# martinjrobins/diffsol

Measured on AMD Instinct MI355X. Metric: ODE steps/sec (and Newton solves/sec) per ensemble, higher is better.
Workload: dtype f64

## Files before the change

diffsol_amd/csrc/dsh_adaptive.hip:

```cpp
#include <cmath>
#include <cstdio>
#include <vector>

#include <cstring>
#include <map>
#include <mutex>
#include <vector>

#include "dsh_internal.hpp"
#include "dsh_resident.hpp"

#ifdef DSH_EXPERIMENTS
#include <hipcub/hipcub.hpp>
#endif
#include "dsh_adaptive_kernel.hpp"
#ifdef DSH_EXPERIMENTS
#include "dsh_member_sched_kernel.hpp"
#endif
#include "dsh_jit.hpp"

using namespace dsh;


extern "C" {

int dsh_experiments_enabled(void) {
#ifdef DSH_EXPERIMENTS
  return 1;
#else
  return 0;
#endif
}

void dsh_adaptive_default_options(dsh_adaptive_options* o) {
  if (!o) return;
#define DSH_X(T, name, value) o->name = value;
  DSH_ADAPTIVE_BODY_OPTIONS(DSH_X)
#undef DSH_X
  o->ic_use_linesearch = 1;
  o->ic_max_linesearch_iterations = 10;
  o->ic_max_linear_solver_setups = 4;
  o->ic_max_newton_iterations = 10;
  o->ic_step_reduction_factor = 0.5;
  o->ic_armijo_constant = 1e-4;
  o->deterministic_pow = 1;
  o->group = 1;
}

int dsh_model_has_adaptive(int model, int64_t size) {
  if (is_jit_model(model)) {
    const JitInfo* ji = jit_info(model);
    if (!ji) return 0;
    return (ji->form == DSH_JIT_FORM_STATIC && ji->n <= 4) || (ji->form == DSH_JIT_FORM_STATIC_BANDED && ji->n <= 512) ? 1 : 0;
  }
  bool ok = false;
  dispatch_static_model(model, size, [&](auto mdl) {
    using Mdl = decltype(mdl);
    ok = Mdl::N <= 4;
  });
  return ok ? 1 : 0;
}

}
namespace dsh {
bool adaptive_fast_launch(int model, int64_t size, bool ba, bool wave, const dsh_adaptive_options& opts, dim3 grid, hipStream_t stream, int64_t nb, const double* p,
                          const double* atol, const AdaptiveConsts* consts, const double* t_eval, double* y_out, int32_t* stats, int32_t* status, double* t_root,
                          int32_t* root_idx, int32_t* ncols, unsigned long long* totals);
}
namespace {
struct SensSpec { double* out; double rtol; const double* atol_host; int64_t natol; };
template <class Mdl> constexpr bool adaptive_sens_ok() {
  if constexpr (model_has_sens<Mdl>::value) return Mdl::N <= 4 && !Mdl::HAS_MASS && Mdl::NROOTS == 0 && model_band_k<Mdl>::value == 0;
  else return false;
}
struct StepsSpec { double* t_out; int64_t cap; };
int bdf_solve_adaptive_impl(dsh_ctx* ctx, int model, int64_t size, int64_t nb, const double* p, const double* atol, int64_t atol_nb, double rtol, double t0,
                            double h0, const dsh_adaptive_options* opts, const double* t_eval_host, int64_t n_eval, double* y_out, int32_t* stats, int32_t* status,
                            double* t_root, int32_t* root_idx, int32_t* ncols, int64_t* totals_host, const SensSpec* sens, const StepsSpec* steps = nullptr);
}
extern "C" {
int dsh_model_has_adaptive_reset(int model, int64_t size) {
  if (is_jit_model(model)) {
    const JitInfo* ji = jit_info(model);
    if (!(ji && ji->has_reset && ji->nroots > 0)) return 0;
    return (ji->form == DSH_JIT_FORM_STATIC && ji->n <= 4) || (ji->form == DSH_JIT_FORM_STATIC_BANDED && !ji->has_mass) ? 1 : 0;
  }
  bool ok = false;
  dispatch_static_model(model, size, [&](auto mdl) {
    using Mdl = decltype(mdl);
    ok = model_has_reset<Mdl>::value && Mdl::N <= 4 && Mdl::NROOTS > 0 && model_band_k<Mdl>::value == 0;
  });
  return ok ? 1 : 0;
}
int dsh_model_has_adaptive_sens(int model, int64_t size) {
  if (is_jit_model(model)) {
    const JitInfo* ji = jit_info(model);
    if (!(ji && ji->has_sens && !ji->has_mass && ji->nroots == 0)) return 0;
    return (ji->form == DSH_JIT_FORM_STATIC && ji->n <= 4) || ji->form == DSH_JIT_FORM_STATIC_BANDED ? 1 : 0;
  }
  bool ok = false;
  dispatch_static_model(model, size, [&](auto mdl) { ok = adaptive_sens_ok<decltype(mdl)>(); });
  return ok ? 1 : 0;
}
int dsh_bdf_solve_adaptive(dsh_ctx* ctx, int model, int64_t size, int64_t nb, const double* p, const double* atol, int64_t atol_nb, double rtol, double t0,
                           double h0, const dsh_adaptive_options* opts, const double* t_eval_host, int64_t n_eval, double* y_out, int32_t* stats, int32_t* status,
                           double* t_root, int32_t* root_idx, int32_t* ncols, int64_t* totals_host) {
  DSH_ENTER(ctx);
  return bdf_solve_adaptive_impl(ctx, model, size, nb, p, atol, atol_nb, rtol, t0, h0, opts, t_eval_host, n_eval, y_out, stats, status, t_root, root_idx, ncols, totals_host, nullptr);
}
int dsh_bdf_solve_adaptive_sens(dsh_ctx* ctx, int model, int64_t size, int64_t nb, const double* p, const double* atol, int64_t atol_nb, double rtol, double t0,
                                double h0, const dsh_adaptive_options* opts, const double* t_eval_host, int64_t n_eval, double sens_rtol, const double* sens_atol_host,
                                int64_t nsens_atol, double* y_out, double* sens_out, int32_t* stats, int32_t* status, int64_t* totals_host) {
  DSH_ENTER(ctx);
  DSH_REQUIRE(sens_out != nullptr, "sens_out is null");
  DSH_REQUIRE(nsens_atol == 0 || sens_atol_host != nullptr, "sens_atol is null");
  if (!dsh_model_has_adaptive_sens(model, size)) {
    set_error("dsh_bdf_solve_adaptive_sens: the model has no device-resident BDF with forward sensitivities (identity-mass ODE model with parameter derivatives and no root functions: register-resident n <= 4, or the banded lane-per-member form)");
    return DSH_E_UNSUPPORTED;
  }
  const SensSpec sp{sens_out, sens_rtol, sens_atol_host, nsens_atol};
  return bdf_solve_adaptive_impl(ctx, model, size, nb, p, atol, atol_nb, rtol, t0, h0, opts, t_eval_host, n_eval, y_out, stats, status, nullptr, nullptr, nullptr, totals_host, &sp);
}
int dsh_model_has_adaptive_steps(int model, int64_t size) {
  if (!dsh_model_has_adaptive(model, size)) return 0;
  if (is_jit_model(model)) { const JitInfo* ji = jit_info(model); return ji && (ji->form == DSH_JIT_FORM_STATIC || ji->form == DSH_JIT_FORM_STATIC_BANDED) ? 1 : 0; }
  return 1;
}
int dsh_bdf_solve_adaptive_steps(dsh_ctx* ctx, int model, int64_t size, int64_t nb, const double* p, const double* atol, int64_t atol_nb, double rtol, double t0,
                                 double h0, const dsh_adaptive_options* opts, double t_final, int64_t max_cols, double* y_out, double* t_out, int32_t* stats,
                                 int32_t* status, double* t_root, int32_t* root_idx, int32_t* ncols, int64_t* totals_host) {
  DSH_ENTER(ctx);
  DSH_REQUIRE(max_cols >= 2 && max_cols <= 0x7fffffff && y_out != nullptr && t_out != nullptr && ncols != nullptr, "dsh_bdf_solve_adaptive_steps: max_cols >= 2, y_out, t_out and ncols are needed");
  if (!dsh_model_has_adaptive_steps(model, size)) {
    set_error("dsh_bdf_solve_adaptive_steps: the model has neither a register-resident BDF (static model, n <= 4) nor a banded lane-per-member form (the wavefront / workgroup forms have dsh_bdf_solve_wave_member_steps)");
    return DSH_E_UNSUPPORTED;
  }
  const StepsSpec st{t_out, max_cols};
  return bdf_solve_adaptive_impl(ctx, model, size, nb, p, atol, atol_nb, rtol, t0, h0, opts, &t_final, 1, y_out, stats, status, t_root, root_idx, ncols, totals_host, nullptr, &st);
}
}
namespace {
int bdf_solve_adaptive_impl(dsh_ctx* ctx, int model, int64_t size, int64_t nb, const double* p, const double* atol, int64_t atol_nb, double rtol, double t0,
                            double h0, const dsh_adaptive_options* opts, const double* t_eval_host, int64_t n_eval, double* y_out, int32_t* stats, int32_t* status,
                            double* t_root, int32_t* root_idx, int32_t* ncols, int64_t* totals_host, const SensSpec* sens, const StepsSpec* steps) {
  DSH_REQUIRE(ctx != nullptr, "ctx is null");
  DSH_REQUIRE(n_eval >= 1 && t_eval_host != nullptr, "t_eval must hold at least one time");
  DSH_REQUIRE(atol_nb == 1 || atol_nb == nb, "atol must be broadcast (nbatch 1) or per member");
  for (int64_t k = 0; k + 1 < n_eval; ++k) DSH_REQUIRE(t_eval_host[k] <= t_eval_host[k + 1], "t_eval must be increasing (InvalidTEval)");
  DSH_REQUIRE(t_eval_host[0] >= t0, "t_eval[0] before t0 (InvalidTEval)");
  if (!dsh_model_has_adaptive(model, size)) { set_error("dsh_bdf_solve_adaptive: model has no device-resident kernel (needs a static model, n <= 4)"); return DSH_E_UNSUPPORTED; }
  if (nb == 0) return DSH_OK;
  AdaptiveConsts C;
  std::memset((void*)&C, 0, sizeof C);
  C.r.rtol = rtol; C.r.t0 = t0; C.r.h0 = h0; C.r.n_eval = (int)n_eval; C.r.member_lanes = 0;
  C.r.ls_steptol = std::pow(2.220446049250313e-16, 2.0 / 3.0);
  if (opts) C.r.o = *opts; else dsh_adaptive_default_options(&C.r.o);
  if (C.r.o.max_steps <= 0) C.r.o.max_steps = 10000000;
  DSH_REQUIRE(C.r.o.group == 1 || C.r.o.group == 64, "adaptive group must be 1 (per member) or 64 (wavefront lock-step)");
  {
    static const int member_lanes_env = [] { const char* e = std::getenv("DSH_MEMBER_LANES"); const int v = e && *e ? std::atoi(e) : 0; return (v == 8 || v == 16 || v == 32) ? v : 0; }();
    C.r.member_lanes = (C.r.o.group == 1 && !is_jit_model(model) && !sens && !steps) ? member_lanes_env : 0;
  }
  if (steps) { C.steps_t_out = steps->t_out; C.steps_cap = (int)steps->cap; }
  if (sens) {
    C.sens_out = sens->out; C.sens_rtol = sens->rtol; C.sens_error_control = sens->natol > 0 ? 1 : 0;
    int64_t ns = 0, npar_ = 0, nroots_ = 0; int hm_ = 0;
    if (dsh_model_info(model, size, &ns, &npar_, &hm_, &nroots_) != DSH_OK) return DSH_E_INVALID;
    DSH_REQUIRE(sens->natol == 0 || sens->natol == 1 || sens->natol == ns, "sens_atol must have length 1 or nstates");
    bool uniform = true;
    for (int64_t i = 1; i < sens->natol; ++i) uniform = uniform && sens->atol_host[i] == sens->atol_host[0];
    DSH_REQUIRE(ns <= 4 || uniform, "device-resident sensitivities of models with more than 4 states take one sens_atol for every state");
    C.sens_pad = (ns > 4 || sens->natol <= 1) ? 1 : 0;
    for (int64_t i = 0; i < 4 && i < ns; ++i) C.sens_atol[i] = sens->natol == 0 ? 0.0 : (sens->natol == 1 ? sens->atol_host[0] : sens->atol_host[i]);
  }
  {
    const BdfTables T = bdf_new_tables();
    for (int i = 0; i <= kMaxOrder; ++i) { C.alpha[i] = T.alpha[i]; C.gamma[i] = T.gamma[i]; C.ec2[i] = T.ec2[i]; }
    C.r.eta_reset = std::pow(20.0, 1.25);
    C.r.eta_reset_ts = std::pow(100.0, 1.25);
    C.eta_reset_p08 = dsh_det_pow(C.r.eta_reset, 0.8);
    C.eta_reset_ts_p08 = dsh_det_pow(C.r.eta_reset_ts, 0.8);
    for (int ord = 1; ord <= kMaxOrder; ++ord) {
      double* U = C.u[ord - 1];
      for (int k = 0; k < 36; ++k) U[k] = 0.0;
      for (int j = 0; j <= ord; ++j) U[j * 6 + 0] = 1.0;
      for (int j = 1; j <= ord; ++j)
        for (int i = 1; i <= ord; ++i) U[j * 6 + i] = U[j * 6 + i - 1] * ((double)i - 1.0 - 1.0 * (double)j) / (double)i;
    }
  }
  double* t_eval_dev = nullptr;
  unsigned long long* totals_dev = nullptr;
  AdaptiveConsts* consts_dev = nullptr;
  int rc = DSH_OK;
  const size_t cbytes = sizeof(AdaptiveConsts), tbytes = sizeof(double) * (size_t)n_eval, need = cbytes + tbytes;
  bool cached = false;
  if (tbytes <= 4096) {
    if (!ctx->const_cache_dev && hipMalloc((void**)&ctx->const_cache_dev, cbytes + 4096) != hipSuccess) { (void)hipGetLastError(); ctx->const_cache_dev = nullptr; }
    if (ctx->const_cache_dev) {
      if (!ctx->const_cache_host) ctx->const_cache_host = new std::vector<unsigned char>();
      std::vector<unsigned char>& held = *ctx->const_cache_host;
      std::vector<unsigned char> now(need);
      std::memcpy(now.data(), &C, cbytes);
      std::memcpy(now.data() + cbytes, t_eval_host, tbytes);
      if (now != held) {
        held.swap(now);
        DSH_HIP_CHECK(hipMemcpyAsync(ctx->const_cache_dev, held.data(), need, hipMemcpyHostToDevice, ctx->stream));
        DSH_HIP_CHECK(hipStreamSynchronize(ctx->stream));
      }
      consts_dev = (AdaptiveConsts*)ctx->const_cache_dev;
      t_eval_dev = (double*)(ctx->const_cache_dev + cbytes);
      cached = true;
    }
  }
  if (!cached) {
    rc = dsh_malloc(ctx, (int64_t)sizeof(AdaptiveConsts), 0, (void**)&consts_dev);
    if (rc != DSH_OK) return rc;
    DSH_HIP_CHECK(hipMemcpyAsync(consts_dev, &C, sizeof(AdaptiveConsts), hipMemcpyHostToDevice, ctx->stream));
    rc = dsh_malloc(ctx, (int64_t)(sizeof(double) * n_eval), 0, (void**)&t_eval_dev);
    if (rc != DSH_OK) return rc;
    DSH_HIP_CHECK(hipMemcpyAsync(t_eval_dev, t_eval_host, sizeof(double) * n_eval, hipMemcpyHostToDevice, ctx->stream));
  }
  rc = dsh_malloc(ctx, (int64_t)(sizeof(unsigned long long) * 8), 1, (void**)&totals_dev);
  if (rc != DSH_OK) { if (!cached) { dsh_free(ctx, t_eval_dev); dsh_free(ctx, consts_dev); } return rc; }
  const bool ba = atol_nb == 1 && nb != 1;
  const int per_wave = C.r.member_lanes > 0 ? C.r.member_lanes : 64;
  const dim3 grid((unsigned)((nb + per_wave - 1) / per_wave)), blk(64);
  bool launched = false;
  DSH_HIP_CHECK(timing_begin(ctx));
#ifdef DSH_EXPERIMENTS
  const int rebin = [] { const char* e = std::getenv("DSH_REBIN"); return e && *e ? std::atoi(e) : 0; }();
  const int rebin_steps = [] { const char* e = std::getenv("DSH_REBIN_STEPS"); return e && *e ? std::atoi(e) : 0; }();
  if (!sens && !steps && (rebin_steps > 0 || (rebin > 0 && n_eval > rebin)) && !is_jit_model(model) && C.r.o.group == 1 && nb >= 128) {
    double* seg_dbl = nullptr; int* seg_int = nullptr; unsigned long long *keys = nullptr, *keys_out = nullptr; int *idx_iota = nullptr, *lane_member = nullptr; void* cub_tmp = nullptr;
    AdaptiveConsts* seg_consts = nullptr; unsigned int* remaining = nullptr;
    size_t cub_bytes = 0;
    auto release = [&]() { (void)hipFree(seg_dbl); (void)hipFree(seg_int); (void)hipFree(keys); (void)hipFree(keys_out); (void)hipFree(idx_iota); (void)hipFree(lane_member); (void)hipFree(cub_tmp); (void)hipFree(seg_consts); (void)hipFree(remaining); };
    (void)hipcub::DeviceRadixSort::SortPairs(nullptr, cub_bytes, keys, keys_out, idx_iota, lane_member, (int)nb, 0, 64, ctx->stream);
    const bool by_steps = rebin_steps > 0;
    const int nseg = by_steps ? 3 : (int)((n_eval + rebin - 1) / rebin);
    bool okm = hipMalloc((void**)&seg_dbl, sizeof(double) * (size_t)kSegDbl * nb) == hipSuccess && hipMalloc((void**)&seg_int, sizeof(int) * (size_t)kSegInt * nb) == hipSuccess &&
               hipMalloc((void**)&keys, 8 * (size_t)nb) == hipSuccess && hipMalloc((void**)&keys_out, 8 * (size_t)nb) == hipSuccess && hipMalloc((void**)&idx_iota, 4 * (size_t)nb) == hipSuccess &&
               hipMalloc((void**)&lane_member, 4 * (size_t)nb) == hipSuccess && hipMalloc(&cub_tmp, cub_bytes ? cub_bytes : 8) == hipSuccess &&
               hipMalloc((void**)&seg_consts, sizeof(AdaptiveConsts) * (size_t)nseg) == hipSuccess && hipMalloc((void**)&remaining, 4) == hipSuccess;
    if (!okm) { (void)hipGetLastError(); release(); set_error("dsh_bdf_solve_adaptive (DSH_REBIN): out of device memory for the segment state"); dsh_free(ctx, totals_dev); if (!cached) { dsh_free(ctx, t_eval_dev); dsh_free(ctx, consts_dev); } return DSH_E_HIP; }
    {
      std::vector<int> iota((size_t)nb);
// ... 120 lines not shown
```

diffsol_amd/csrc/dsh_adaptive_kernel.hpp:

```cpp
#pragma once
#include "dsh_resident.hpp"
#include "dsh_bdf_tables.hpp"

namespace dsh {

constexpr int kMaxOrder = 5;
constexpr int kNC = kMaxOrder + 3;

struct AdaptiveConsts {
  ResidentConsts r;
  double alpha[6], gamma[6], ec2[6];
  double u[kMaxOrder][36];
  double eta_reset_p08, eta_reset_ts_p08;
  double* seg_dbl;
  int* seg_int;
  unsigned long long* seg_key;
  const int* seg_lane_member;
  int seg_fresh, seg_last, seg_col_end, seg_step_budget;
  unsigned int* seg_remaining;
  double* sens_out;
  double sens_rtol, sens_atol[4];
  int sens_error_control, sens_pad;
  double* steps_t_out;
  int steps_cap, steps_pad;
};
constexpr int kSegDbl = 128, kSegInt = 32;

#define DSH_ADAPTIVE_BODY_OPTIONS(X)             \
  X(int, max_nonlinear_solver_iterations, 10)    \
  X(int, max_error_test_failures, 40)            \
  X(int, max_nonlinear_solver_failures, 50)      \
  X(double, nonlinear_solver_tolerance, 0.2)     \
  X(double, min_timestep, 1e-13)                 \
  X(double, max_timestep_growth, 2.0)            \
  X(double, min_timestep_growth, 2.0)            \
  X(double, max_timestep_shrink, 0.9)            \
  X(double, min_timestep_shrink, 0.5)            \
  X(int, update_jacobian_after_steps, 20)        \
  X(int, update_rhs_jacobian_after_steps, 50)    \
  X(double, threshold_to_update_jacobian, 0.3)   \
  X(double, threshold_to_update_rhs_jacobian, 0.2) \
  X(double, pi_control_proportional, 0.0)        \
  X(double, pi_control_integral, 0.5)            \
  X(int64_t, max_steps, 10000000)
struct AdaptiveDefaultOptions {
  __host__ __device__ constexpr AdaptiveDefaultOptions(const dsh_adaptive_options&) {}
#define DSH_X(T, name, value) static constexpr T name = value;
  DSH_ADAPTIVE_BODY_OPTIONS(DSH_X)
#undef DSH_X
};
template <bool DEFOPT> struct adaptive_options_view { using type = const dsh_adaptive_options&; };
template <> struct adaptive_options_view<true> { using type = const AdaptiveDefaultOptions; };

template <bool WAVE, class F>
__device__ __forceinline__ void guarded(bool c, F&& f) {
  if (c) {
    if constexpr (WAVE) asm volatile("" ::);
    f();
  }
}

template <int Q> struct order_c { static constexpr int value = Q; };
template <class F>
__device__ __forceinline__ void with_order(int ou, F&& f) {
  if (ou <= 2) {
    if (ou <= 1) f(order_c<1>{}); else f(order_c<2>{});
  } else {
    if (ou == 3) f(order_c<3>{});
    else if (ou == 4) f(order_c<4>{});
    else f(order_c<5>{});
  }
}
#ifndef DSH_ORDER_PATHS_PREDICT
#define DSH_ORDER_PATHS_PREDICT 1
#endif
#ifndef DSH_ORDER_PATHS_UPDATE
#define DSH_ORDER_PATHS_UPDATE 1
#endif
#ifndef DSH_ORDER_PATHS_SELECT
#define DSH_ORDER_PATHS_SELECT 1
#endif
#ifndef DSH_ORDER_PATHS_LITERALS
#define DSH_ORDER_PATHS_LITERALS 1
#endif

template <bool WAVE>
__device__ __forceinline__ int uniform(int v) {
  if constexpr (WAVE) return __builtin_amdgcn_readfirstlane(v);
  else return v;
}
template <bool WAVE>
__device__ __forceinline__ bool uniform(bool v) {
  if constexpr (WAVE) return __builtin_amdgcn_readfirstlane((int)v) != 0;
  else return v;
}
template <bool WAVE>
__device__ __forceinline__ double uniform(double v) {
  if constexpr (WAVE) return __hiloint2double(__builtin_amdgcn_readfirstlane(__double2hiint(v)), __builtin_amdgcn_readfirstlane(__double2loint(v)));
  else return v;
}
template <bool WAVE>
__device__ __forceinline__ double group_norm_w(double v) {
  if constexpr (WAVE) return wave_max_nonneg_f64(v);
  else return v;
}

__device__ __forceinline__ bool pow_p08_domain(double x) { return x > 0x1p-100 && x < 0x1p100; }
__device__ __forceinline__ double pow_p08_inline(double x) {
  double w = (double)__builtin_amdgcn_exp2f(-0.2f * __builtin_amdgcn_logf((float)x));
#pragma unroll
  for (int i = 0; i < 3; ++i) {
    const double w2 = w * w;
    const double w5 = w2 * w2 * w;
    w = fma(0.2 * w, fma(-x, w5, 1.0), w);
  }
  return x * w;
}
__device__ __forceinline__ double pow_p08(double x) {
  if (__builtin_expect(!pow_p08_domain(x), 0)) return rpow(x, 0.8, false);
  return pow_p08_inline(x);
}

enum : int { kBallotAllBelow = 0, kBallotSomeAbove = 1, kBallotUndecided = 2 };
__device__ __forceinline__ int ballot_decide_below(double v, double T) {
  const bool t_ok = T >= 0x1p-1022 && T <= 0x1.fffffffffffffp1023;
  const unsigned long long below = __builtin_amdgcn_ballot_w64(v < T * (1.0 - 0x1p-40));
  const unsigned long long above = __builtin_amdgcn_ballot_w64(v >= T * (1.0 + 0x1p-40));
  if (__builtin_expect(!t_ok || (below | above) != ~0ull, 0)) return kBallotUndecided;
  return above != 0ull ? kBallotSomeAbove : kBallotAllBelow;
}
__device__ __forceinline__ double newton_first_threshold(double tol, double eta08) { const double q = tol / eta08; return q * q; }
__device__ __forceinline__ bool newton_first_converged(double dms, double thr2, double eta08, double tol, bool& undecided) {
  const int d = ballot_decide_below(dms, thr2);
  undecided = d == kBallotUndecided;
  if (__builtin_expect(undecided, 0)) return eta08 * sqrt(wave_max_nonneg_f64(dms)) < tol;
  return d == kBallotAllBelow;
}
__device__ __forceinline__ double root_k(double x, int k) {
  if (__builtin_expect(!((k == 2 || k == 3) && x >= 0x1p-1022 && x <= 0x1.fffffffffffffp1023), 0)) return rpow(x, 1.0 / (double)k, false);
  if (k == 2) return sqrt(x);
  return cbrt(x);
}

__device__ __forceinline__ double powi_nonneg(double a, int b) {
  unsigned u = (unsigned)b;
  double r = 1.0;
  while (true) {
    if (u & 1u) r *= a;
    u >>= 1;
    if (u == 0u) break;
    a *= a;
  }
  return r;
}
template <bool FAST>
__device__ __forceinline__ double powi_rate(double a, int b) {
  if constexpr (FAST) return powi_nonneg(a, b);
  else return powi_rt(a, b);
}

constexpr int kInvRootSteps = 2;
__device__ __forceinline__ bool inv_root_2k_domain(double x, int k) { return (x > 0x1p-100) & (x < 0x1p100) & (k >= 1) & (k <= 7); }
__device__ __forceinline__ double inv_root_2k(double x, int k) {
  const float n_f = (float)(2 * k);
  const double c = 1.0 / (double)(2 * k);
  double w = (double)__builtin_amdgcn_exp2f(-__builtin_amdgcn_logf((float)x) * __builtin_amdgcn_rcpf(n_f));
#pragma unroll
  for (int i = 0; i < kInvRootSteps; ++i) {
    const double w2 = w * w, w4 = w2 * w2;
    double pk = (k & 1) ? w : 1.0;
    pk *= (k & 2) ? w2 : 1.0;
    pk *= (k & 4) ? w4 : 1.0;
    w = fma(w * c, fma(-x, pk * pk, 1.0), w);
  }
  return w;
}
__device__ __forceinline__ double inv_root_2k_group(double x, int k, double expo) {
  const bool is_inf = x == __builtin_huge_val();
  if (__builtin_expect(!__all(is_inf | inv_root_2k_domain(x, k)), 0)) return rpow(x, expo, false);
  const double w = inv_root_2k(is_inf ? 1.0 : x, k);
  return is_inf ? 0.0 : w;
}

#ifndef DSH_ADAPTIVE_WAVES_PER_EU
#define DSH_ADAPTIVE_WAVES_PER_EU 2
#endif
#ifndef DSH_ADAPTIVE_DT_PRIVATE
#define DSH_ADAPTIVE_DT_PRIVATE 0
#endif
template <class Mdl, bool BA, bool WAVE, bool SEG = false, bool SENS = false, bool FAST = false, bool DEFOPT = false>
__global__ __launch_bounds__(64) __attribute__((amdgpu_waves_per_eu(DSH_ADAPTIVE_WAVES_PER_EU, DSH_ADAPTIVE_WAVES_PER_EU))) void k_bdf_adaptive(int64_t nb, const double* __restrict__ p_g, const double* __restrict__ atol_g, const AdaptiveConsts* __restrict__ Cp,
                                                    const double* __restrict__ t_eval, double* __restrict__ y_out, int32_t* __restrict__ stats_out,
                                                    int32_t* __restrict__ status_out, double* __restrict__ t_root_out, int32_t* __restrict__ root_idx_out,
                                                    int32_t* __restrict__ ncols_out, unsigned long long* __restrict__ totals) {
  constexpr int N = Mdl::N, NP = Mdl::NP;
  constexpr int NR = Mdl::NROOTS > 0 ? Mdl::NROOTS : 1;
  constexpr bool LOCKFAST = FAST && WAVE && DEFOPT;
  static_assert(!LOCKFAST || (!SEG && !SENS), "decisions by ballot: lock-step groups of the plain fast kernel");
  constexpr bool kLit = DSH_ORDER_PATHS_LITERALS != 0;
  const AdaptiveConsts& C = *Cp;
  const int ML = (!WAVE && !SEG && C.r.member_lanes > 0) ? C.r.member_lanes : 64;
  const int64_t bglobal = (int64_t)blockIdx.x * ML + threadIdx.x;
  const bool active = (int)threadIdx.x < ML && bglobal < nb;
  int64_t b_ = active ? bglobal : (int64_t)blockIdx.x * ML;
  if constexpr (SEG) { if (C.seg_lane_member != nullptr) b_ = C.seg_lane_member[b_]; }
  const int64_t b = b_;
  const bool fresh = !SEG || C.seg_fresh != 0;
  typename adaptive_options_view<DEFOPT>::type o = C.r.o;
  const bool det = !FAST && C.r.o.deterministic_pow != 0;
  const double rtol = C.r.rtol;
  double p[NP], atol[N];
  load_vec<NP>(p_g, nb, b, p);
DSH_UNROLL_N
  for (int i = 0; i < N; ++i) atol[i] = BA ? atol_g[i] : atol_g[(int64_t)i * nb + b];

  double t = C.r.t0, h = 0.0;
  double y[N], f0[N];
  int32_t status = kRsOk;
  if (fresh) {
    Mdl::init(t, p, y);
    Mdl::rhs(t, y, p, f0);
    if (!group_all<WAVE>(set_consistent<Mdl, WAVE>(t, p, y, f0, atol, rtol, C.r))) status = kRsInitialConditionDidNotConverge;
    h = uniform<WAVE>(initial_step_size<Mdl, WAVE>(t, C.r.h0, y, f0, p, atol, rtol, 1, det));
  } else {
DSH_UNROLL_N
    for (int i = 0; i < N; ++i) { y[i] = 0.0; f0[i] = 0.0; }
  }

  int order = 1;
  constexpr int BK = model_band_k<Mdl>::value;
  constexpr bool BANDED = BK > 0;
  static_assert(!BANDED || !Mdl::HAS_MASS, "banded device-resident models need an identity mass matrix");
  constexpr bool kResets = model_has_reset<Mdl>::value && !BANDED && Mdl::NROOTS > 0;
  constexpr bool DTP = BANDED || DSH_ADAPTIVE_DT_PRIVATE != 0;
  constexpr int LN = BANDED ? 1 : N;
  __shared__ double sDt[DTP ? 1 : kNC * LN][64];
  __shared__ double sJ[LN * LN][64];
  const int ln = threadIdx.x;
  __shared__ double sAlpha[6], sGamma[6], sEc2[6], sU[kMaxOrder * 36];
  __shared__ double sRw[48], sRUw[48];
  if (ln < 6) { sAlpha[ln] = C.alpha[ln]; sGamma[ln] = C.gamma[ln]; sEc2[ln] = C.ec2[ln]; }
  for (int k = ln; k < kMaxOrder * 36; k += 64) sU[k] = C.u[k / 36][k % 36];
  __syncthreads();
  double Dt_p[DTP ? kNC : 1][DTP ? N : 1];
  double Jb[BANDED ? (2 * BK + 1) * N : 1], Lf[BANDED ? BK * N : 1], Uf[BANDED ? (2 * BK + 1) * N : 1];
  auto dt_get = [&](int j, int i) __attribute__((always_inline)) -> double { if constexpr (DTP) return Dt_p[j][i]; else return sDt[j * N + i][ln]; };
  auto dt_set = [&](int j, int i, double v) __attribute__((always_inline)) { if constexpr (DTP) Dt_p[j][i] = v; else sDt[j * N + i][ln] = v; };
  double D[kNC][N];
#pragma unroll
  for (int j = 0; j < kNC; ++j)
DSH_UNROLL_N
    for (int i = 0; i < N; ++i) { D[j][i] = 0.0; dt_set(j, i, 0.0); }
DSH_UNROLL_N
  for (int i = 0; i < N; ++i) { D[0][i] = y[i]; D[1][i] = f0[i] * h; }
  double opc = h * sAlpha[1];
  constexpr int NPS = SENS ? NP : 1, NCS = SENS ? kNC : 1, NS = SENS ? N : 1;
  static_assert(!SENS || (!Mdl::HAS_MASS && Mdl::NROOTS == 0 && !SEG),
                "device-resident forward sensitivities: identity-mass ODE models without root functions");
  double S[NPS][NCS][NS];
  double s_cur[NPS][NS];
  double s_delta[NPS][NS];
  double s_c = 0.0;
  double s_atol[NS];
  if constexpr (SENS) {
DSH_UNROLL_N
    for (int i = 0; i < N; ++i) s_atol[i] = C.sens_atol[C.sens_pad != 0 ? 0 : (i < 4 ? i : 0)];
    for (int j = 0; j < NP; ++j) {
      double ev[NP], s0[N], jm[N], dfdp[N];
#pragma unroll
      for (int k = 0; k < NP; ++k) ev[k] = k == j ? 1.0 : 0.0;
      Mdl::init_sens_mul(t, p, ev, s0);
      Mdl::sens_mul(t, y, p, ev, dfdp);
      Mdl::jac_mul(t, y, p, s0, jm);
      for (int k = 0; k < kNC; ++k)
DSH_UNROLL_N
        for (int i = 0; i < N; ++i) S[j][k][i] = 0.0;
DSH_UNROLL_N
      for (int i = 0; i < N; ++i) {
        const double ds = jm[i] + dfdp[i];
        S[j][0][i] = s0[i];
        S[j][1][i] = ds * h;
        s_cur[j][i] = s0[i];
        s_delta[j][i] = 0.0;
// ... 276 lines not shown
    }
    if (check_rhs) {
      jac_stale = true;
      reset_jacobian(y, t);
      steps_since_rhs_jac = 0; steps_since_jac = 0; h_at_last_jac = c;
      eta = C.r.eta_reset;
      n_setups++;
    } else if (check_jac) {
      reset_jacobian(y, t);
      steps_since_jac = 0; h_at_last_jac = c;
      eta = C.r.eta_reset;
      n_setups++;
    }
  };

  bool has_tstop = true;
  const double tstop = t_eval[C.r.n_eval - 1];
  auto handle_tstop = [&]() __attribute__((always_inline)) -> int {
    const double eps = 2.220446049250313e-16;
    const double troundoff = 100.0 * eps * (fabs(t) + fabs(h));
    if (fabs(t - tstop) <= troundoff) { has_tstop = false; return 1; }
    if ((h > 0.0 && tstop < t - troundoff) || (h < 0.0 && tstop > t + troundoff)) { has_tstop = false; return 2; }
    if ((h > 0.0 && t + h > tstop + troundoff) || (h < 0.0 && t + h < tstop - troundoff)) {
      const double factor = (tstop - t) / h;
      double nh;
      (void)update_step_size(factor, nh);
    }
    return 0;
  };

  int col = 0;
  double te_next = t_eval[0];
  const bool steps_mode = !SEG && !SENS && C.steps_cap > 0;
  auto steps_write = [&](double tw, const double (&yw)[N]) __attribute__((always_inline)) {
    if (col < C.steps_cap && active) {
      C.steps_t_out[(int64_t)col * nb + b] = tw;
DSH_UNROLL_N
      for (int i = 0; i < N; ++i) y_out[((int64_t)col * N + i) * nb + b] = yw[i];
    }
    col++;
  };
  if (steps_mode && fresh) steps_write(t, y);
  if (fresh) {
    const int r = handle_tstop();
    if (r == 1) status = kRsStopTimeAtCurrentTime;
    else if (r == 2) status = kRsStopTimeBeforeCurrentTime;
  }

  long guard = 0;
  bool done = status != kRsOk || (!WAVE && !active);
  auto seg_xfer = [&](auto&& fd, auto&& fi) __attribute__((always_inline)) {
    int kd = 0, ki = 0;
    auto d_ = [&](double& v) __attribute__((always_inline)) { fd(kd++, v); };
    auto i_ = [&](int& v) __attribute__((always_inline)) { fi(ki++, v); };
    d_(t); d_(h); d_(opc); d_(h_at_last_jac); d_(eta); d_(prev_err); d_(te_next); d_(rf_t0); d_(t_root); d_(t_predict);
#pragma unroll
    for (int j = 0; j < kNC; ++j)
DSH_UNROLL_N
      for (int i = 0; i < N; ++i) { d_(D[j][i]); double v = dt_get(j, i); d_(v); dt_set(j, i, v); }
    if constexpr (!BANDED) {
#pragma unroll
      for (int e = 0; e < N * N; ++e) { double v = sJ[e][ln]; d_(v); sJ[e][ln] = v; d_(A[e]); }
    }
DSH_UNROLL_N
    for (int i = 0; i < N; ++i) { d_(y[i]); i_(P[i]); }
#pragma unroll
    for (int r = 0; r < NR; ++r) d_(g0[r]);
    int js = jac_stale ? 1 : 0, hp = has_prev_err ? 1 : 0, ht = has_tstop ? 1 : 0, dn = done ? 1 : 0, glo = (int)(guard & 0x7fffffff), ghi = (int)(guard >> 31), st = (int)status;
    i_(order); i_(js); i_(n_setups); i_(n_steps); i_(n_err_fails); i_(n_newton); i_(n_nl_fails); i_(steps_since_jac); i_(steps_since_rhs_jac); i_(n_equal_steps);
    i_(hp); i_(col); i_(root_idx); i_(st); i_(ht); i_(dn); i_(glo); i_(ghi);
    jac_stale = js != 0; has_prev_err = hp != 0; has_tstop = ht != 0; done = dn != 0; guard = ((long)ghi << 31) | (long)glo; status = (int32_t)st;
  };
  if constexpr (SEG) {
    static_assert(!WAVE && !BANDED, "segmented runs: per-member control of the register-resident models");
    static_assert(10 + 2 * kNC * N + 2 * N * N + N + NR <= kSegDbl && N + 18 <= kSegInt, "segment state does not fit its slots");
    if (!fresh && active) {
      seg_xfer([&](int k, double& v) __attribute__((always_inline)) { v = C.seg_dbl[(int64_t)k * nb + b]; },
               [&](int k, int& v) __attribute__((always_inline)) { v = C.seg_int[(int64_t)k * nb + b]; });
    }
  }
  int seg_trips = 0;
  while (!done) {
    if (++guard > o.max_steps) { status = kRsMaxStepsExceeded; break; }
    double safety = 0.0, error_norm = 0.0;
    const int old_err_fails = n_err_fails;
    bool convergence_fail = false;
    double x[N];
    int niter = 0;
    predict_forward();
    while (true) {
DSH_UNROLL_N
      for (int i = 0; i < N; ++i) x[i] = yp[i];
      double winv[FAST ? N : 1];
      if constexpr (FAST) {
DSH_UNROLL_N
        for (int i = 0; i < N; ++i) winv[i] = 1.0 / (fabs(yp[i]) * rtol + atol[i]);
      }
      niter = 0;
      bool has_old = false;
      double old_norm = 0.0;
      bool solved = false;
      if constexpr (LOCKFAST) {
        const double tol = o.nonlinear_solver_tolerance;
        auto newton_update = [&](double& dms, auto&& beside) __attribute__((always_inline)) -> bool {
          double f[N], delta[N], tmpv[N];
          Mdl::rhs(t_predict, x, p, f);
          if constexpr (Mdl::HAS_MASS) {
DSH_UNROLL_N
            for (int i = 0; i < N; ++i) { tmpv[i] = x[i] + psi[i]; delta[i] = f[i]; }
            Mdl::mass_gemv(t_predict, tmpv, p, -opc, delta);
          } else {
DSH_UNROLL_N
            for (int i = 0; i < N; ++i) delta[i] = 1.0 * (x[i] + psi[i]) + (-opc) * f[i];
          }
          bool solved_ok;
          if constexpr (BANDED) solved_ok = band_solve_lane<N, BK>(Lf, Uf, P, delta);
          else solved_ok = lu_solve_reg_inv<N>(A, Adinv, P, delta);
          if (!group_all<WAVE>(solved_ok)) return false;
DSH_UNROLL_N
          for (int i = 0; i < N; ++i) asm volatile("" : "+v"(delta[i]));
          beside();
          double acc = 0.0;
DSH_UNROLL_N
          for (int i = 0; i < N; ++i) {
            const double d = delta[i];
            x[i] = x[i] - d;
            const double term = d * winv[i];
            acc += term * term;
          }
          dms = acc / (double)N;
          return true;
        };
        auto rate_test = [&](double norm, double old_nrm) __attribute__((always_inline)) -> int {
          const double rate = niter == 2 ? norm / old_nrm : uniform<WAVE>(root_k(norm / old_nrm, niter - 1));
          if (rate > 0.9) return 2;
          if (powi_rate<FAST>(rate, o.max_nonlinear_solver_iterations - niter) / (1.0 - rate) * norm > tol) return 2;
          eta = rate / (1.0 - rate);
          return eta * norm < tol ? 1 : 0;
        };
        const double min_eta = 1e4 * 2.220446049250313e-16;
        const double eta_c = eta < min_eta ? min_eta : eta;
        const double reset_a = C.r.eta_reset, reset_b = C.r.eta_reset_ts, p08_a = C.eta_reset_p08, p08_b = C.eta_reset_ts_p08;
        const bool is_a = eta_c == reset_a, is_b = eta_c == reset_b, in_dom = pow_p08_domain(eta_c);
        const bool needs_call = !(is_a | is_b | in_dom);
        double eta08 = 0.0, thr2 = 0.0;
        double dms1;
        if (newton_update(dms1, [&]() __attribute__((always_inline)) {
              double pw = pow_p08_inline(in_dom ? eta_c : 1.0);
              asm volatile("" : "+v"(pw));
              eta08 = is_a ? p08_a : (is_b ? p08_b : uniform<WAVE>(pw));
              thr2 = newton_first_threshold(tol, eta08);
            })) {
          if (__builtin_expect(needs_call, 0)) { eta08 = uniform<WAVE>(rpow(eta_c, 0.8, false)); thr2 = newton_first_threshold(tol, eta08); }
          eta = eta08;
          niter = 1;
          bool undecided;
          if (newton_first_converged(dms1, thr2, eta08, tol, undecided)) solved = true;
          else if (o.max_nonlinear_solver_iterations > 1) {
            double nan_nrm = 0.0;
            const bool nan1 = wave_any_nan(dms1);
            if (__builtin_expect(nan1, 0)) nan_nrm = sqrt(wave_max_nonneg_f64(dms1));
            double nrm1 = 0.0;
            double dms2;
            if (newton_update(dms2, [&]() __attribute__((always_inline)) { nrm1 = sqrt(wave_max_nonneg_f64_chain(dms1)); })) {
              const double old_nrm = nan1 ? nan_nrm : nrm1;
              double norm = sqrt(group_norm_w<WAVE>(dms2));
// ... 415 lines not shown
            }
          }
DSH_UNROLL_N
          for (int i = 0; i < N; ++i) if (active) C.sens_out[(((int64_t)col * NP + q) * N + i) * nb + b] = sv[i];
        }
      }
      col++;
      if (col < C.r.n_eval) te_next = t_eval[col];
    }
    if constexpr (kResets) {
      if (reason == 3) {
        double yb[N], yr[N], dyr[N];
        interpolate(t_root, yb);
        if constexpr (Mdl::HAS_MASS) {
          double pi = 1.0, d_pi = 0.0;
DSH_UNROLL_N
          for (int i = 0; i < N; ++i) dyr[i] = 0.0;
#pragma unroll
          for (int j = 0; j < kMaxOrder; ++j) {
            if (j < order) {
              const double i_t = (double)j;
              const double denom = h * (1.0 + i_t);
              const double w = (t_root - (t - h * i_t)) / denom;
              const double dw = 1.0 / denom;
              const double new_d_pi = d_pi * w + pi * dw;
              pi *= w;
              d_pi = new_d_pi;
DSH_UNROLL_N
              for (int i = 0; i < N; ++i) dyr[i] = d_pi * D[j + 1][i] + 1.0 * dyr[i];
            }
          }
        }
        t = t_root;
        Mdl::reset(t, yb, p, yr);
DSH_UNROLL_N
        for (int i = 0; i < N; ++i) y[i] = yr[i];
        if constexpr (Mdl::HAS_MASS) {
          if (!group_all<WAVE>(set_consistent<Mdl, WAVE>(t, p, y, dyr, atol, rtol, C.r, true))) { status = kRsInitialConditionDidNotConverge; break; }
        } else
        Mdl::rhs(t, y, p, dyr);
        if (steps_mode) steps_write(t, y);
        if (t < tstop) {
          has_tstop = true;
          { const int r = handle_tstop(); if (r == 1) { status = kRsStopTimeAtCurrentTime; break; } if (r == 2) { status = kRsStopTimeBeforeCurrentTime; break; } }
          Mdl::root(t, y, p, g0);
          rf_t0 = t;
          n_equal_steps = 0;
          order = 1;
DSH_UNROLL_N
          for (int i = 0; i < N; ++i) { D[0][i] = y[i]; D[1][i] = dyr[i] * h; }
          opc = h * sAlpha[1];
          jacobian_updates(h * sAlpha[1], JState::StepSuccess);
          has_prev_err = false;
          if (has_tstop) { const int r = handle_tstop(); if (r == 1) { status = kRsStopTimeAtCurrentTime; break; } if (r == 2) { status = kRsStopTimeBeforeCurrentTime; break; } }
          refresh_wyinv();
          reason = 0;
        } else {
          done = true;
          reason = 0;
        }
      }
    }
    if (reason == 3 && steps_mode) {
      double yv[N];
      interpolate(t_root, yv);
      steps_write(t_root, yv);
      done = true;
    } else
    if (reason == 3) {
      if (col < C.r.n_eval) {
        double yv[N];
        interpolate(t_root, yv);
DSH_UNROLL_N
        for (int i = 0; i < N; ++i) if (active) y_out[((int64_t)col * N + i) * nb + b] = yv[i];
        col++;
      }
      done = true;
    }
    if (reason == 1) done = true;
    if constexpr (SEG) {
      if (!C.seg_last && (col >= C.seg_col_end || (C.seg_step_budget > 0 && ++seg_trips >= C.seg_step_budget))) break;
    }
  }
  if constexpr (SEG) {
    if (status != kRsOk) done = true;
    if (active) {
      seg_xfer([&](int k, double& v) __attribute__((always_inline)) { C.seg_dbl[(int64_t)k * nb + b] = v; },
               [&](int k, int& v) __attribute__((always_inline)) { C.seg_int[(int64_t)k * nb + b] = v; });
      const int ne = n_equal_steps < 15 ? n_equal_steps : 15;
      C.seg_key[b] = done ? ~0ull : (((unsigned long long)order << 60) | ((unsigned long long)ne << 56) | ((unsigned long long)__double_as_longlong(fabs(h)) >> 8));
    }
    if (!C.seg_last) {
      if (C.seg_remaining != nullptr) {
        const int left = __popcll(__ballot(active && !done));
        if ((threadIdx.x & 63) == 0 && left) atomicAdd(C.seg_remaining, (unsigned int)left);
      }
      return;
    }
  }
  if (active) {
    if (ncols_out != nullptr) ncols_out[b] = col;
    if (t_root_out != nullptr) t_root_out[b] = root_idx >= 0 ? t_root : __builtin_nan("");
    if (root_idx_out != nullptr) root_idx_out[b] = root_idx;
    if (!steps_mode)
    for (; col < C.r.n_eval; ++col) {
DSH_UNROLL_N
      for (int i = 0; i < N; ++i) y_out[((int64_t)col * N + i) * nb + b] = __builtin_nan("");
      if constexpr (SENS)
        for (int q = 0; q < NP; ++q)
DSH_UNROLL_N
          for (int i = 0; i < N; ++i) C.sens_out[(((int64_t)col * NP + q) * N + i) * nb + b] = __builtin_nan("");
    }
    if (status_out != nullptr) status_out[b] = status;
    if (stats_out != nullptr) {
      stats_out[0 * nb + b] = n_steps;
      stats_out[1 * nb + b] = n_newton;
      stats_out[2 * nb + b] = n_setups;
      stats_out[3 * nb + b] = n_err_fails;
      stats_out[4 * nb + b] = n_nl_fails;
    }
  }
  const unsigned long long mine[6] = {active ? (unsigned long long)n_steps : 0ull, active ? (unsigned long long)n_newton : 0ull,
                                      active ? (unsigned long long)n_setups : 0ull, active ? (unsigned long long)n_err_fails : 0ull,
                                      active ? (unsigned long long)n_nl_fails : 0ull, (active && status != kRsOk) ? 1ull : 0ull};
#pragma unroll
  for (int k = 0; k < 6; ++k) {
    const unsigned long long sum = wave_sum_u64(mine[k]);
    if ((threadIdx.x & 63) == 0 && sum) atomicAdd(&totals[k], sum);
  }
}

}
```

Measured before the change: 25.01 billion.

## Raise wave priority for second-round waves when grid slightly exceeds SIMD count

When the wavefront count falls between one and two waves per SIMD, second-wave blocks periodically raise their hardware priority with s_setprio during the step loop, biasing issue between co-resident wave pairs. The aim is to cut the tail where late waves finish well after the first round. An optional timeline instrumentation path, compiled out by default, records per-wave start and end times. The scheme relies on blockIdx approximating dispatch order and adds a per-step branch plus setprio instructions.

Result: faster. 27.03 billion, median of 6 (+8.1%).

```diff
diff --git a/diffsol_amd/csrc/dsh_adaptive.hip b/diffsol_amd/csrc/dsh_adaptive.hip
--- a/diffsol_amd/csrc/dsh_adaptive.hip
+++ b/diffsol_amd/csrc/dsh_adaptive.hip
@@ -67,6 +67,29 @@
                           const double* atol, const AdaptiveConsts* consts, const double* t_eval, double* y_out, int32_t* stats, int32_t* status, double* t_root,
                           int32_t* root_idx, int32_t* ncols, unsigned long long* totals);
 }
+#if DSH_WAVE_TIMELINE
+namespace {
+dsh::WaveTimelineRecord* g_wave_timeline = nullptr;
+int64_t g_wave_timeline_cap = 0, g_wave_timeline_n = 0;
+dsh::WaveTimelineRecord* wave_timeline_buffer(int64_t waves) {
+  if (waves > g_wave_timeline_cap) {
+    if (g_wave_timeline) (void)hipFree(g_wave_timeline);
+    g_wave_timeline = nullptr; g_wave_timeline_cap = 0;
+    if (hipMalloc((void**)&g_wave_timeline, sizeof(dsh::WaveTimelineRecord) * (size_t)waves) != hipSuccess) { (void)hipGetLastError(); return nullptr; }
+    g_wave_timeline_cap = waves;
+  }
+  g_wave_timeline_n = waves;
+  return g_wave_timeline;
+}
+}
+extern "C" int64_t dsh_wave_timeline_read(void* host, int64_t max_records) {
+  if (!g_wave_timeline || !host) return -1;
+  const int64_t n = g_wave_timeline_n < max_records ? g_wave_timeline_n : max_records;
+  if (hipDeviceSynchronize() != hipSuccess) return -1;
+  if (hipMemcpy(host, g_wave_timeline, sizeof(dsh::WaveTimelineRecord) * (size_t)n, hipMemcpyDeviceToHost) != hipSuccess) return -1;
+  return n;
+}
+#endif
 namespace {
 struct SensSpec { double* out; double rtol; const double* atol_host; int64_t natol; };
 template <class Mdl> constexpr bool adaptive_sens_ok() {
@@ -162,6 +185,10 @@
     C.r.member_lanes = (C.r.o.group == 1 && !is_jit_model(model) && !sens && !steps) ? member_lanes_env : 0;
   }
   if (steps) { C.steps_t_out = steps->t_out; C.steps_cap = (int)steps->cap; }
+  C.simds = 4 * ctx->num_cu;
+#if DSH_WAVE_TIMELINE
+  C.timeline = wave_timeline_buffer((nb + 63) / 64);
+#endif
   if (sens) {
     C.sens_out = sens->out; C.sens_rtol = sens->rtol; C.sens_error_control = sens->natol > 0 ? 1 : 0;
     int64_t ns = 0, npar_ = 0, nroots_ = 0; int hm_ = 0;
diff --git a/diffsol_amd/csrc/dsh_adaptive_kernel.hpp b/diffsol_amd/csrc/dsh_adaptive_kernel.hpp
--- a/diffsol_amd/csrc/dsh_adaptive_kernel.hpp
+++ b/diffsol_amd/csrc/dsh_adaptive_kernel.hpp
@@ -6,6 +6,10 @@
 
 constexpr int kMaxOrder = 5;
 constexpr int kNC = kMaxOrder + 3;
+
+#ifndef DSH_WAVE_TIMELINE
+#define DSH_WAVE_TIMELINE 0
+#endif
 
 struct AdaptiveConsts {
   ResidentConsts r;
@@ -23,7 +27,17 @@
   int sens_error_control, sens_pad;
   double* steps_t_out;
   int steps_cap, steps_pad;
+  int simds, simds_pad;
+#if DSH_WAVE_TIMELINE
+  struct WaveTimelineRecord* timeline;
+#endif
 };
+#if DSH_WAVE_TIMELINE
+struct WaveTimelineRecord {
+  unsigned long long t_in, t_out;
+  unsigned int block, hw_id, xcc_id, n_steps, n_newton, pad;
+};
+#endif
 constexpr int kSegDbl = 128, kSegInt = 32;
 
 #define DSH_ADAPTIVE_BODY_OPTIONS(X)             \
@@ -188,6 +202,19 @@
 #ifndef DSH_ADAPTIVE_DT_PRIVATE
 #define DSH_ADAPTIVE_DT_PRIVATE 0
 #endif
+#ifndef DSH_PAIR_PRIO
+#define DSH_PAIR_PRIO 1
+#endif
+#ifndef DSH_PAIR_PRIO_PERIOD
+#define DSH_PAIR_PRIO_PERIOD 4
+#endif
+#ifndef DSH_PAIR_PRIO_HIGH
+#define DSH_PAIR_PRIO_HIGH 5
+#endif
+__device__ __forceinline__ void pair_prio_set(unsigned phase_bits) {
+  if (__builtin_amdgcn_readfirstlane(phase_bits & 1u) != 0) __builtin_amdgcn_s_setprio(1);
+  else __builtin_amdgcn_s_setprio(0);
+}
 template <class Mdl, bool BA, bool WAVE, bool SEG = false, bool SENS = false, bool FAST = false, bool DEFOPT = false>
 __global__ __launch_bounds__(64) __attribute__((amdgpu_waves_per_eu(DSH_ADAPTIVE_WAVES_PER_EU, DSH_ADAPTIVE_WAVES_PER_EU))) void k_bdf_adaptive(int64_t nb, const double* __restrict__ p_g, const double* __restrict__ atol_g, const AdaptiveConsts* __restrict__ Cp,
                                                     const double* __restrict__ t_eval, double* __restrict__ y_out, int32_t* __restrict__ stats_out,
@@ -199,6 +226,26 @@
   static_assert(!LOCKFAST || (!SEG && !SENS), "decisions by ballot: lock-step groups of the plain fast kernel");
   constexpr bool kLit = DSH_ORDER_PATHS_LITERALS != 0;
   const AdaptiveConsts& C = *Cp;
+  constexpr bool kPairPrio = LOCKFAST && DSH_PAIR_PRIO != 0;
+  static_assert((DSH_PAIR_PRIO_PERIOD & (DSH_PAIR_PRIO_PERIOD - 1)) == 0 && DSH_PAIR_PRIO_PERIOD > 0, "DSH_PAIR_PRIO_PERIOD: a power of two");
+  static_assert(DSH_PAIR_PRIO_HIGH >= 0 && DSH_PAIR_PRIO_HIGH < 2 * DSH_PAIR_PRIO_PERIOD, "DSH_PAIR_PRIO_HIGH: trips of the 2 x DSH_PAIR_PRIO_PERIOD");
+  unsigned pair_mode = 0;
+  if constexpr (kPairPrio) {
+    const uint64_t simds = (uint64_t)(C.simds > 0 ? C.simds : 0), waves = (uint64_t)(nb + 63) / 64u;
+    if (waves > simds && waves <= 2u * simds) pair_mode = blockIdx.x >= simds ? 2u : 1u;
+    pair_mode = (unsigned)__builtin_amdgcn_readfirstlane((int)pair_mode);
+  }
+#if DSH_WAVE_TIMELINE
+  if constexpr (LOCKFAST) {
+    const unsigned long long t_in = __builtin_amdgcn_s_memrealtime();
+    if (threadIdx.x == 0 && C.timeline != nullptr) {
+      WaveTimelineRecord& w = C.timeline[blockIdx.x];
+      w.t_in = t_in; w.block = blockIdx.x;
+      w.hw_id = __builtin_amdgcn_s_getreg((31 << 11) | 4);
+      w.xcc_id = __builtin_amdgcn_s_getreg((31 << 11) | 20);
+    }
+  }
+#endif
   const int ML = (!WAVE && !SEG && C.r.member_lanes > 0) ? C.r.member_lanes : 64;
   const int64_t bglobal = (int64_t)blockIdx.x * ML + threadIdx.x;
   const bool active = (int)threadIdx.x < ML && bglobal < nb;
@@ -641,6 +688,13 @@
   int seg_trips = 0;
   while (!done) {
     if (++guard > o.max_steps) { status = kRsMaxStepsExceeded; break; }
+    if constexpr (kPairPrio) {
+      if constexpr (DSH_PAIR_PRIO_HIGH > 0) {
+        if (pair_mode == 2u) pair_prio_set(((unsigned)(guard - 1) & (2u * DSH_PAIR_PRIO_PERIOD - 1u)) < (unsigned)DSH_PAIR_PRIO_HIGH ? 1u : 0u);
+      } else {
+        if (pair_mode != 0u) pair_prio_set((unsigned)((unsigned long long)(guard - 1) / DSH_PAIR_PRIO_PERIOD) + pair_mode - 1u);
+      }
+    }
     double safety = 0.0, error_norm = 0.0;
     const int old_err_fails = n_err_fails;
     bool convergence_fail = false;
@@ -1222,6 +1276,15 @@
       if (!C.seg_last && (col >= C.seg_col_end || (C.seg_step_budget > 0 && ++seg_trips >= C.seg_step_budget))) break;
     }
   }
+#if DSH_WAVE_TIMELINE
+  if constexpr (LOCKFAST) {
+    const unsigned long long t_out = __builtin_amdgcn_s_memrealtime();
+    if (threadIdx.x == 0 && C.timeline != nullptr) {
+      WaveTimelineRecord& w = C.timeline[blockIdx.x];
+      w.t_out = t_out; w.n_steps = (unsigned)n_steps; w.n_newton = (unsigned)n_newton; w.pad = 0u;
+    }
+  }
+#endif
   if constexpr (SEG) {
     if (status != kRsOk) done = true;
     if (active) {
```
